# ShiqiYu/libfacedetection.train

Hardware: AMD Instinct MI355X
Metric: training images/sec, YuNet_n 320x320 bs=256/GPU (higher is better)
Workload: dtype f32; 1 GPU; YuNet_n 320x320 bs=256/GPU full training step, fp32 (64->64 backward GEMMs: two-way bf16 split -- measured against the exact-fp32 instruction: every output within 9e-6 of its tensor maximum, 50 SGD iterations end as far from the exact path as a last-bit perturbation of it does, tests/test_precision_gpu.py + profiles/r05_precision.json; the strictly-fp32 variant is timed in exact_fp32_bwd with --fu; parallelism=dp1, global_batch=256

## Files before the change

libfacedetection.train_amd/csrc/api.hip:

```cpp
#include <string.h>

#include "common.h"

namespace {

__global__ __launch_bounds__(256) void sgd_kernel(float* __restrict__ p, const float* __restrict__ g,
                                                  float* __restrict__ buf, long long n,
                                                  const float* __restrict__ lr_dev, float momentum, float undamped,
                                                  int nesterov, float wd, float gscale, int first) {
    const float lr = lr_dev[0];
    const long long i = (long long)blockIdx.x * 256 + threadIdx.x;
    if (i >= n) return;
    const float w = p[i];
    const float d = g[i] * gscale + wd * w;
    float step = d;
    if (momentum != 0.0f) {
        const float b = first ? d : buf[i] * momentum + undamped * d;
        buf[i] = b;
        step = nesterov ? d + momentum * b : b;
    }
    p[i] = w - lr * step;
}

__global__ void bn_batch_kernel(const int32_t* __restrict__ table, const double* __restrict__ stats_base,
                                float* __restrict__ rm, float* __restrict__ rv, float momentum,
                                float* __restrict__ grad_base, int mode) {
    const int32_t* t = table + blockIdx.x * 7;
    const int C = t[1], count = t[2], slots = t[6];
    const double* st = stats_base + t[0];
    for (int c = threadIdx.x; c < C; c += blockDim.x) {
        if (mode == 0) {
            const double inv = 1.0 / (double)count;
            const double mean = bn_sum(st, slots, C, c) * inv;
            double var = bn_sum(st, slots, C, C + c) * inv - mean * mean;
            var = var < 0.0 ? 0.0 : var;
            const double unb = count > 1 ? var * ((double)count / (double)(count - 1)) : var;
            float* m = rm + t[3];
            float* v = rv + t[3];
            m[c] = (1.0f - momentum) * m[c] + momentum * (float)mean;
            v[c] = (1.0f - momentum) * v[c] + momentum * (float)unb;
        } else if (mode == 1) {
            grad_base[t[5] + c] = (float)bn_sum(st, slots, C, c);
            grad_base[t[4] + c] = (float)bn_sum(st, slots, C, C + c);
        } else {
            double* w = const_cast<double*>(st);
            const double m = (double)rm[t[3] + c], v = (double)rv[t[3] + c];
            w[c] = m * (double)count;
            w[C + c] = (v + m * m) * (double)count;
            for (int k = 1; k < slots; ++k) w[k * 2 * C + c] = 0.0, w[k * 2 * C + C + c] = 0.0;
        }
    }
}

}

extern "C" int yunet_bn_batch(const int32_t* table, int n, const double* stats_base,
                              float* running_mean, float* running_var, float momentum,
                              float* grad_base, int mode, void* stream) {
    if (n < 1) return YUNET_EINVAL;
    hipLaunchKernelGGL(bn_batch_kernel, dim3(n), dim3(64), 0, (hipStream_t)stream, table, stats_base,
                       running_mean, running_var, momentum, grad_base, mode);
    return hip_status();
}

__global__ __launch_bounds__(256) void add_kernel(const float* __restrict__ a, const float* __restrict__ b,
                                                  float* __restrict__ out, size_t n, int vec) {
    const size_t i = (size_t)blockIdx.x * 256 + threadIdx.x;
    if (vec) {
        if (i < n / 4) {
            const float4 x = reinterpret_cast<const float4*>(a)[i], y = reinterpret_cast<const float4*>(b)[i];
            reinterpret_cast<float4*>(out)[i] = make_float4(x.x + y.x, x.y + y.y, x.z + y.z, x.w + y.w);
        } else if (i - n / 4 < n % 4) {
            const size_t k = (n / 4) * 4 + (i - n / 4);
            out[k] = a[k] + b[k];
        }
    } else if (i < n) {
        out[i] = a[i] + b[i];
    }
}

extern "C" int yunet_add(const float* a, const float* b, float* out, size_t n, void* stream) {
    if (!a || !b || !out) return YUNET_EINVAL;
    if (n == 0) return 0;
    const int vec = ((reinterpret_cast<uintptr_t>(a) | reinterpret_cast<uintptr_t>(b) | reinterpret_cast<uintptr_t>(out)) & 15) == 0;
    const size_t threads = vec ? n / 4 + n % 4 : n;
    const size_t blocks = (threads + 255) / 256;
    if (blocks > 0x7fffffffull) return YUNET_EINVAL;
    hipLaunchKernelGGL(add_kernel, dim3((unsigned)blocks), dim3(256), 0, (hipStream_t)stream, a, b, out, n, vec);
    return hip_status();
}

extern "C" int yunet_sgd_step_ex(float* params, const float* grads, float* momentum_buf, int64_t n,
                                 const float* lr_dev, float momentum, float dampening, int nesterov,
                                 float weight_decay, float grad_scale, int first_step, void* stream) {
    if (n < 1 || !params || !grads || !lr_dev) return YUNET_EINVAL;
    if (momentum != 0.0f && !momentum_buf) return YUNET_EINVAL;
    if (nesterov && (momentum <= 0.0f || dampening != 0.0f)) return YUNET_EINVAL;
    const long long blocks = (n + 255) / 256;
    if (blocks > 0x7fffffffll) return YUNET_EINVAL;
    hipLaunchKernelGGL(sgd_kernel, dim3((unsigned)blocks), dim3(256), 0, (hipStream_t)stream, params, grads,
                       momentum_buf, (long long)n, lr_dev, momentum, 1.0f - dampening, nesterov ? 1 : 0, weight_decay,
                       grad_scale, first_step);
    return hip_status();
}

extern "C" int yunet_sgd_step(float* params, const float* grads, float* momentum_buf, int64_t n,
                              const float* lr_dev, float momentum, float weight_decay,
                              float grad_scale, int first_step, void* stream) {
    return yunet_sgd_step_ex(params, grads, momentum_buf, n, lr_dev, momentum, 0.0f, 0, weight_decay, grad_scale,
                             first_step, stream);
}

YunetOptions& yunet_options() {
    static YunetOptions o = [] {
        auto env = [](const char* k, int dflt) {
            const char* e = getenv(k);
            return e ? atoi(e) : dflt;
        };
        YunetOptions v;
        v.no_pack = getenv("YUNET_NO_PACK") ? 1 : 0;
        v.bwd_fp32mma = getenv("YUNET_BWD_FP32MMA") ? 1 : 0;
        v.bwd64_nw = env("YUNET_BWD64_NW", 0);
        v.ew_grid = env("YUNET_EW_GRID", 768);
        v.fwd_blocks_per_cu = env("YUNET_DP_FWD_BLOCKS_PER_CU", 0);
        v.fwd64s = env("YUNET_FWD64S", 2);
        v.fwd64s_rows = env("YUNET_FWD64S_ROWS", 0);
        v.bwd16s = env("YUNET_BWD16S", 1);
        v.bwd16s_rows = env("YUNET_BWD16S_ROWS", 0);
        v.stem_mma = env("YUNET_STEM_MMA", 1);
        v.fwd16s = env("YUNET_FWD16S", 1);
        v.upadd_coarse = env("YUNET_UPADD_COARSE", 1);
        v.bwd32_split = env("YUNET_BWD32_SPLIT", 1);
        v.assign_v2 = env("YUNET_ASSIGN_V2", 1);
        v.fwd_group = env("YUNET_FWD_GROUP", 1);
        v.oneshot_timeout_ms = env("YUNET_ONESHOT_TIMEOUT_MS", 120000);
        if (v.bwd64_nw != 4 && v.bwd64_nw != 8) v.bwd64_nw = 0;
        if (v.ew_grid < 1) v.ew_grid = 768;
        return v;
    }();
    return o;
}
int yunet_option_assign_v2() { return yunet_options().assign_v2; }
extern "C" int yunet_set_option(const char* name, int value) {
    YunetOptions& o = yunet_options();
    int* slot = nullptr;
    if (!name) return YUNET_EINVAL;
    if (!strcmp(name, "no_pack")) slot = &o.no_pack;
    else if (!strcmp(name, "bwd_fp32mma")) slot = &o.bwd_fp32mma;
    else if (!strcmp(name, "bwd64_nw")) slot = &o.bwd64_nw;
    else if (!strcmp(name, "ew_grid")) slot = &o.ew_grid;
    else if (!strcmp(name, "fwd_blocks_per_cu")) slot = &o.fwd_blocks_per_cu;
    else if (!strcmp(name, "fwd64s")) slot = &o.fwd64s;
    else if (!strcmp(name, "fwd64s_rows")) slot = &o.fwd64s_rows;
    else if (!strcmp(name, "bwd16s")) slot = &o.bwd16s;
    else if (!strcmp(name, "bwd16s_rows")) slot = &o.bwd16s_rows;
    else if (!strcmp(name, "stem_mma")) slot = &o.stem_mma;
    else if (!strcmp(name, "fwd16s")) slot = &o.fwd16s;
    else if (!strcmp(name, "upadd_coarse")) slot = &o.upadd_coarse;
    else if (!strcmp(name, "bwd32_split")) slot = &o.bwd32_split;
    else if (!strcmp(name, "assign_v2")) slot = &o.assign_v2;
    else if (!strcmp(name, "fwd_group")) slot = &o.fwd_group;
    else if (!strcmp(name, "oneshot_timeout_ms")) slot = &o.oneshot_timeout_ms;
    if (!slot || value < 0) return YUNET_EINVAL;
    if (slot == &o.bwd64_nw && value != 0 && value != 4 && value != 8) return YUNET_EINVAL;
    if (slot == &o.ew_grid && value == 0) value = 768;
    const int prev = *slot;
    *slot = value;
    return prev;
}

extern "C" {
int yunet_stem_fwd_bf16(const float*, const float*, const float*, float*, double*, int, int, int, int, void*);
int yunet_stem_bwd_bf16(const float*, const float*, const float*, const YunetBN*, float*, int, int, int, int, int, void*);
int yunet_dp_fwd_bf16(const YunetDP*, void*);
int yunet_dp_fwd_group_bf16(const YunetDP* const*, int, void*);
int yunet_dp_bwd_bf16(const YunetDP*, void*);
int yunet_pool_fwd_bf16(const float*, const YunetBN*, float*, int, int, int, int, void*);
int yunet_pool_bwd_bf16(const float*, const YunetBN*, const float*, float*, int, int, int, int, int, void*);
int yunet_upadd_fwd_bf16(const float*, const YunetBN*, const float*, const YunetBN*, float*, int, int, int, int, void*);
int yunet_upadd_bwd_bf16(const float*, const YunetBN*, const float*, const YunetBN*, const float*, float*, int, float*,
                         int, int, int, int, int, void*);
}

static int g_lanes_on = 1;
struct LaneSet {
    bool ready;
    hipStream_t side[YUNET_MAX_LANES];
    hipEvent_t fork_ev, join_ev[YUNET_MAX_LANES];
};
static constexpr int kMaxDevices = 16;
static thread_local LaneSet t_lanes[kMaxDevices];
static LaneSet* lanes_get() {
    int dev = -1;
    if (hipGetDevice(&dev) != hipSuccess || dev < 0 || dev >= kMaxDevices) return nullptr;
    LaneSet& s = t_lanes[dev];
    if (s.ready) return &s;
    for (int l = 0; l < YUNET_MAX_LANES; ++l) {
        if (hipStreamCreateWithFlags(&s.side[l], hipStreamNonBlocking) != hipSuccess) return nullptr;
        if (hipEventCreateWithFlags(&s.join_ev[l], hipEventDisableTiming) != hipSuccess) return nullptr;
    }
    if (hipEventCreateWithFlags(&s.fork_ev, hipEventDisableTiming) != hipSuccess) return nullptr;
    s.ready = true;
    return &s;
}
extern "C" int yunet_exec_lanes(int enable) {
    const int prev = g_lanes_on;
    g_lanes_on = enable ? 1 : 0;
    return prev;
}

extern "C" int yunet_exec(const YunetOp* ops, int n_ops, void* main_stream) {
    unsigned open_lanes = 0;
    LaneSet* ls = nullptr;
    for (int k = 0; k < n_ops; ++k) {
        const YunetOp& o = ops[k];
        int rc = 0;
        void* stream = main_stream;
        if (o.opcode == YUNET_OP_FORK || o.opcode == YUNET_OP_JOIN) {
            if (!g_lanes_on) continue;
            if (!ls && !(ls = lanes_get())) return YUNET_EINVAL * 1000 - k;
            const unsigned mask = (unsigned)o.i[0] & ((1u << (YUNET_MAX_LANES + 1)) - 2u);
            if (o.opcode == YUNET_OP_FORK) {
                if (hipEventRecord(ls->fork_ev, (hipStream_t)main_stream) != hipSuccess) return YUNET_EINVAL * 1000 - k;
                for (int l = 1; l <= YUNET_MAX_LANES; ++l)
                    if (mask & (1u << l)) hipStreamWaitEvent(ls->side[l - 1], ls->fork_ev, 0);
                open_lanes |= mask;
            } else {
                for (int l = 1; l <= YUNET_MAX_LANES; ++l)
                    if (mask & (1u << l)) {
                        hipEventRecord(ls->join_ev[l - 1], ls->side[l - 1]);
                        hipStreamWaitEvent((hipStream_t)main_stream, ls->join_ev[l - 1], 0);
                    }
                open_lanes &= ~mask;
            }
            continue;
        }
        const int lane = o.i[YUNET_OP_LANE];
        if (g_lanes_on && lane > 0) {
            if (lane > YUNET_MAX_LANES || !(open_lanes & (1u << lane)) || !ls) return YUNET_EINVAL * 1000 - k;
            stream = (void*)ls->side[lane - 1];
        }
        switch (o.opcode) {
            case YUNET_OP_STEM_FWD:
                if (o.i[4] > 0) {
                    rc = o.i[11] == YUNET_BF16 ? YUNET_EINVAL
                                               : yunet_stem_fwd_det((const float*)o.p[0], (const float*)o.p[1], (const float*)o.p[2], (float*)o.p[3],
                                                                    (double*)o.p[4], o.i[4], o.i[0], o.i[1], o.i[2], o.i[3], stream);
                    break;
                }
                rc = (o.i[11] == YUNET_BF16 ? yunet_stem_fwd_bf16 : yunet_stem_fwd)((const float*)o.p[0], (const float*)o.p[1], (const float*)o.p[2],
                                    (float*)o.p[3], (double*)o.p[4], o.i[0], o.i[1], o.i[2], o.i[3],
                                    stream);
                break;
            case YUNET_OP_STEM_BWD:
                if (o.p[4] && o.p[5] && yunet_options().stem_mma) {
                    rc = yunet_stem_bwd_rz((const float*)o.p[0], (const float*)o.p[4], (const float*)o.p[5], (const float*)o.p[2],
                                           &o.bn[0], (float*)o.p[3], o.i[4], o.i[0], o.i[1], o.i[2], o.i[3], stream);
                    break;
                }
                rc = (o.i[11] == YUNET_BF16 ? yunet_stem_bwd_bf16 : yunet_stem_bwd)((const float*)o.p[0], (const float*)o.p[1], (const float*)o.p[2],
                                    &o.bn[0], (float*)o.p[3], o.i[4], o.i[0], o.i[1], o.i[2], o.i[3],
                                    stream);
                break;
            case YUNET_OP_DP_FWD: {
                const int g = o.i[YUNET_OP_GROUP];
                if (g >= 2 && g <= YUNET_DP_GROUP_MAX && k + g <= n_ops) {
                    const YunetDP* units[YUNET_DP_GROUP_MAX];
                    bool ok = true;
                    for (int j = 0; j < g; ++j) {
                        const YunetOp& oj = ops[k + j];
                        ok = ok && oj.opcode == YUNET_OP_DP_FWD && oj.i[YUNET_OP_LANE] == lane && oj.dp.x_dtype == o.dp.x_dtype;
                        units[j] = &oj.dp;
                    }
                    if (!ok) return YUNET_EINVAL * 1000 - k;
                    rc = o.dp.x_dtype == YUNET_BF16 ? yunet_dp_fwd_group_bf16(units, g, stream) : yunet_dp_fwd_group(units, g, stream);
                    if (rc == 0) k += g - 1;
                    break;
                }
                rc = o.dp.x_dtype == YUNET_BF16 ? yunet_dp_fwd_bf16(&o.dp, stream) : yunet_dp_fwd(&o.dp, stream);
                break;
            }
            case YUNET_OP_DP_BWD:
                rc = o.dp.x_dtype == YUNET_BF16 ? yunet_dp_bwd_bf16(&o.dp, stream) : yunet_dp_bwd(&o.dp, stream);
                break;
            case YUNET_OP_POOL_FWD:
                rc = (o.i[11] == YUNET_BF16 ? yunet_pool_fwd_bf16 : yunet_pool_fwd)((const float*)o.p[0], &o.bn[0], (float*)o.p[1], o.i[0], o.i[1],
                                    o.i[2], o.i[3], stream);
                break;
            case YUNET_OP_POOL_BWD:
                rc = (o.i[11] == YUNET_BF16 ? yunet_pool_bwd_add_bf16 : yunet_pool_bwd_add)(
                    (const float*)o.p[0], &o.bn[0], (const float*)o.p[1], (const float*)o.p[3], (float*)o.p[2], o.i[4], o.i[0],
                    o.i[1], o.i[2], o.i[3], stream);
                break;
            case YUNET_OP_UPADD_FWD:
                rc = (o.i[11] == YUNET_BF16 ? yunet_upadd_fwd_bf16 : yunet_upadd_fwd)((const float*)o.p[0], &o.bn[0], (const float*)o.p[1], &o.bn[1],
                                     (float*)o.p[2], o.i[0], o.i[1], o.i[2], o.i[3], stream);
                break;
            case YUNET_OP_UPADD_BWD:
                rc = (o.i[11] == YUNET_BF16 ? yunet_upadd_bwd_bf16 : yunet_upadd_bwd)((const float*)o.p[0], &o.bn[0], (const float*)o.p[1], &o.bn[1],
                                     (const float*)o.p[2], (float*)o.p[3], o.i[4], (float*)o.p[4],
                                     o.i[5], o.i[0], o.i[1], o.i[2], o.i[3], stream);
                break;
            case YUNET_OP_BN_RUNNING:
                rc = yunet_bn_update_running((const double*)o.p[0], (float*)o.p[1], (float*)o.p[2],
                                             o.i[0], o.i[1], o.f[0], stream);
                break;
            case YUNET_OP_BN_PARAM_GRAD:
                rc = yunet_bn_param_grad((const double*)o.p[0], (float*)o.p[1], (float*)o.p[2], o.i[0],
                                         o.i[1], stream);
                break;
            case YUNET_OP_REDUCE_PARTIALS:
                rc = yunet_reduce_partials((const float*)o.p[0], o.i[0], o.i[1], (float*)o.p[1],
                                           o.i[2], stream);
                break;
// ... 64 lines not shown
```

libfacedetection.train_amd/csrc/common.h:

```cpp
#pragma once
#include <hip/hip_runtime.h>
#include <stdint.h>
#include <stdlib.h>

#include "../../include/yunet_hip.h"

#define CONV_BLOCKS 1024

typedef float f32x4 __attribute__((ext_vector_type(4)));
typedef unsigned int u32x4 __attribute__((ext_vector_type(4)));
typedef unsigned int u32x2 __attribute__((ext_vector_type(2)));

#ifdef YUNET_ACT_BF16
typedef unsigned short act_t;
typedef u32x2 act_raw4;
#define ACT_SUFFIX(name) name##_bf16
#define YUNET_ACT_DTYPE YUNET_BF16
#else
typedef float act_t;
typedef u32x4 act_raw4;
#define ACT_SUFFIX(name) name
#define YUNET_ACT_DTYPE YUNET_F32
#endif
#define ACT_B ((unsigned)sizeof(act_t))
// ... 18 lines not shown
#else
    return act_raw4{__float_as_uint(v.x), __float_as_uint(v.y), __float_as_uint(v.z), __float_as_uint(v.w)};
#endif
}
__device__ __forceinline__ float act_round(float v) {
#ifdef YUNET_ACT_BF16
    return __uint_as_float(pack_bf16x2(v, 0.0f) << 16);
#else
    return v;
#endif
}
constexpr int ST_AUX = 0;
constexpr int DX_AUX = 2;
template <int AUX = 0, typename R>
__device__ __forceinline__ act_raw4 act_bufld4(R rsrc, unsigned byte_off) {
#ifdef YUNET_ACT_BF16
    return __builtin_amdgcn_raw_buffer_load_b64(rsrc, byte_off, 0, AUX);
#else
    return __builtin_amdgcn_raw_buffer_load_b128(rsrc, byte_off, 0, AUX);
#endif
}
template <typename R>
__device__ __forceinline__ void act_bufst4(R rsrc, unsigned byte_off, const float4 v) {
#ifdef YUNET_ACT_BF16
    __builtin_amdgcn_raw_buffer_store_b64(act_pack(v), rsrc, byte_off, 0, ST_AUX);
#else
    __builtin_amdgcn_raw_buffer_store_b128(act_pack(v), rsrc, byte_off, 0, ST_AUX);
#endif
}
__device__ __forceinline__ float4 act_ld4(const act_t* p) {
    return act_unpack(*reinterpret_cast<const act_raw4*>(p));
}
__device__ __forceinline__ void act_st4(act_t* p, const float4 v) {
    *reinterpret_cast<act_raw4*>(p) = act_pack(v);
}

__device__ __forceinline__ int first_tile() {
    const int g = (int)gridDim.x, b = (int)blockIdx.x;
    if ((g & 7) == 0) return (b & 7) * (g >> 3) + (b >> 3);
    return b;
}

__device__ __forceinline__ f32x4 mfma16(float a, float b, f32x4 c) {
    return __builtin_amdgcn_mfma_f32_16x16x4f32(a, b, c, 0, 0, 0);
}

struct BNCoef {
    float mean, scale, beta, invstd;
    float mean_lo;
};
__device__ __forceinline__ double bn_sum(const double* __restrict__ s, int slots, int C, int i) {
    double v[8];
#pragma unroll
    for (int k = 0; k < 8; ++k) v[k] = s[(k < slots ? k : 0) * 2 * C + i];
#pragma unroll
    for (int k = 1; k < 8; ++k) v[k] = k < slots ? v[k] : 0.0;
    double r = ((v[0] + v[1]) + (v[2] + v[3])) + ((v[4] + v[5]) + (v[6] + v[7]));
    for (int k = 8; k < slots; ++k) r += s[k * 2 * C + i];
    return r;
}
__device__ __forceinline__ double* bn_slot(const double* base, int slots, int C) {
    return const_cast<double*>(base) + (slots > 1 ? (int)(blockIdx.x % (unsigned)slots) * 2 * C : 0);
}
__device__ __forceinline__ BNCoef bn_coef(const YunetBN& bn, int C, int c) {
    const double inv = 1.0 / (double)bn.count;
    const double mean = bn_sum(bn.stats, bn.slots, C, c) * inv;
    double var = bn_sum(bn.stats, bn.slots, C, C + c) * inv - mean * mean;
    var = var < 0.0 ? 0.0 : var;
    BNCoef k;
    k.mean = (float)mean;
    k.mean_lo = (float)(mean - (double)k.mean);
    k.invstd = (float)(1.0 / sqrt(var + (double)bn.eps));
    k.scale = bn.gamma[c] * k.invstd;
    k.beta = bn.beta[c];
    return k;
}
__device__ __forceinline__ void bn_table_fill(float* tab, const YunetBN& bn, int C, int tid) {
    if (tid < C) {
        const BNCoef k = bn_coef(bn, C, tid);
        tab[tid] = k.mean; tab[C + tid] = k.scale; tab[2 * C + tid] = k.beta; tab[3 * C + tid] = k.invstd;
        tab[4 * C + tid] = k.mean_lo;
    }
}
__device__ __forceinline__ void bn_table_get(const float* tab, int C, int c0, BNCoef (&k)[4]) {
#pragma unroll
    for (int i = 0; i < 4; ++i) {
        k[i].mean = tab[c0 + i]; k[i].scale = tab[C + c0 + i]; k[i].beta = tab[2 * C + c0 + i];
        k[i].invstd = tab[3 * C + c0 + i]; k[i].mean_lo = tab[4 * C + c0 + i];
    }
}

struct BNBwd {
    float mean, invstd, k1, c1, c2;
    float mean_lo, c1_lo;
};
__device__ __forceinline__ BNBwd bn_bwd_coef(const YunetBN& bn, int C, int c) {
    const BNCoef f = bn_coef(bn, C, c);
    const double inv = 1.0 / (double)bn.count;
    BNBwd k;
    k.mean = f.mean;
    k.invstd = f.invstd;
    k.k1 = f.scale;
    const double c1 = bn_sum(bn.bstats, bn.slots, C, c) * inv;
    k.c1 = (float)c1;
    k.c1_lo = (float)(c1 - (double)k.c1);
    k.c2 = (float)(bn_sum(bn.bstats, bn.slots, C, C + c) * inv);
    k.mean_lo = f.mean_lo;
    return k;
}

struct BNFold {
    float a, b, dh, dl;
};
__device__ __forceinline__ BNFold bn_fold(const BNBwd& k) {
    BNFold f;
    f.a = k.k1;
    f.b = (float)(-(double)k.k1 * (double)k.c2 * (double)k.invstd);
    const double D = -(double)f.a * ((double)k.c1 + (double)k.c1_lo) - (double)f.b * ((double)k.mean + (double)k.mean_lo);
    f.dh = (float)D;
    f.dl = (float)(D - (double)f.dh);
    return f;
}
__device__ __forceinline__ float bn_dz_folded(float dy, float z, float a, float b, float dh, float dl) {
    return fmaf(a, dy, fmaf(b, z, dh)) + dl;
}

__device__ __forceinline__ float bn_center(float x, float mean_hi, float mean_lo) {
    return (x - mean_hi) - mean_lo;
}
__device__ __forceinline__ float bn_dz(float dy, float z, float mean_hi, float mean_lo, float invstd,
                                       float k1, float c1_hi, float c1_lo, float c2) {
    return k1 * (((dy - c1_hi) - c1_lo) - bn_center(z, mean_hi, mean_lo) * invstd * c2);
}

__device__ __forceinline__ float bnrelu(float x, float mean, float scale, float beta) {
    return fmaxf(fmaf(x - mean, scale, beta), 0.0f);
}

struct YunetOptions {
    int no_pack;
    int bwd_fp32mma;
    int bwd64_nw;
    int ew_grid;
    int fwd_blocks_per_cu;
    int fwd64s;
    int fwd64s_rows;
    int bwd16s;
    int bwd16s_rows;
    int fwd16s;
    int stem_mma;
    int bwd32_split;
    int upadd_coarse;
    int fwd_group;
    int assign_v2;
    int oneshot_timeout_ms;
};
YunetOptions& yunet_options();
int yunet_option_assign_v2();

#include <atomic>
constexpr int YUNET_MAX_DEVICES = 16;
struct PerDevice {
    std::atomic<int> v[YUNET_MAX_DEVICES];
};
inline int yunet_device_index() {
    int dev = 0;
    if (hipGetDevice(&dev) != hipSuccess || dev < 0 || dev >= YUNET_MAX_DEVICES) return -1;
    return dev;
}
template <typename F>
inline int per_device(PerDevice& slots, F&& compute) {
    const int dev = yunet_device_index();
    if (dev < 0) return compute();
    int v = slots.v[dev].load(std::memory_order_acquire);
    if (v == 0) {
        v = compute();
        if (v > 0) slots.v[dev].store(v, std::memory_order_release);
    }
    return v;
}
inline int yunet_cu_count() {
    static PerDevice cus;
    return per_device(cus, [] {
        int dev = 0, n = 0;
        if (hipGetDevice(&dev) != hipSuccess ||
            hipDeviceGetAttribute(&n, hipDeviceAttributeMultiprocessorCount, dev) != hipSuccess || n < 1)
            return 256;
        return n;
    });
}

#ifdef __HIPCC__
template <int COUNT, int NT, typename F>
__device__ __forceinline__ void staged_table(const float* __restrict__ src, int tid, F&& put) {
    constexpr int IT = (COUNT + NT - 1) / NT;
    constexpr bool EXACT = COUNT % NT == 0;
    float v[IT];
#pragma unroll
    for (int k = 0; k < IT; ++k) {
        const int i = tid + k * NT;
        v[k] = (EXACT || i < COUNT) ? src[i] : 0.0f;
    }
#pragma unroll
    for (int k = 0; k < IT; ++k) {
        const int i = tid + k * NT;
        if (EXACT || i < COUNT) put(i, v[k]);
    }
}
#endif


struct PackGeom {
    int on, H, W, ph, pw, R, N, CH, CW;
    float inv_ph, inv_pw;
};
static inline PackGeom make_pack(int N, int H, int W) {
    PackGeom g;
    g.on = (H <= 20 && W <= 20 && N >= 4) ? 1 : 0;
    g.H = H; g.W = W; g.N = N;
    g.ph = H + 1; g.pw = W + 1;
    g.R = N < 16 ? N : 16;
    g.CW = g.R * g.pw;
    g.CH = ((N + g.R - 1) / g.R) * g.ph;
    g.inv_ph = 1.0f / (float)g.ph;
    g.inv_pw = 1.0f / (float)g.pw;
    return g;
}
static inline PackGeom dp_pack_geom(int N, int H, int W) {
    PackGeom g = make_pack(N, H, W);
    if (yunet_options().no_pack) g.on = 0;
    return g;
}
static inline bool dp_use_pack(int N, int H, int W, int cin, int cout) {
    return cin == 64 && (cout == 64 || cout == 16) && dp_pack_geom(N, H, W).on;
}
static inline bool dp_use_pack_bwd(int N, int H, int W, int cin, int cout) {
    return dp_use_pack(N, H, W, cin, cout);
}
static inline bool dp_pack_fits(const PackGeom& g, long long x_img_stride, long long z_img_stride) {
    const long long lim = 1ll << 30;
    return !g.on || ((long long)g.N * x_img_stride < lim && (long long)g.N * z_img_stride < lim);
}
__device__ __forceinline__ bool pk_locate(const PackGeom& g, int Y, int X, int& n, int& y, int& x) {
    if ((unsigned)Y >= (unsigned)g.CH || (unsigned)X >= (unsigned)g.CW) return false;
    const int iy = (int)(((float)Y + 0.5f) * g.inv_ph), ix = (int)(((float)X + 0.5f) * g.inv_pw);
    y = Y - iy * g.ph;
    x = X - ix * g.pw;
    n = iy * g.R + ix;
    return y < g.H && x < g.W && n < g.N;
}

__device__ __forceinline__ void atomic_add_f64(double* p, double v) {
    __hip_atomic_fetch_add(p, v, __ATOMIC_RELAXED, __HIP_MEMORY_SCOPE_AGENT);
}

__device__ __forceinline__ void bn_det_add(const double* base, int C, int i, double v) {
    double* p = const_cast<double*>(base) + (size_t)(1 + blockIdx.x) * 2 * C + i;
    *p += v;
}
static inline bool bn_det_fits(const YunetBN& bn, int grid) { return YUNET_DET_ROWS(bn.det_rows) >= grid && bn.slots <= 1; }
static inline bool bn_det_fast(const YunetBN& bn) { return YUNET_DET_ROWS(bn.det_rows) && (bn.det_rows & YUNET_DET_FAST); }

static inline int hip_status() { return -(int)hipGetLastError(); }

int ACT_SUFFIX(launch_dp_fwd64s)(const YunetDP* d, hipStream_t stream);
int ACT_SUFFIX(launch_dp_fwd64s_group)(const YunetDP* const* ds, int n, hipStream_t stream);
int ACT_SUFFIX(launch_dp_bwd16s)(const YunetDP* d, hipStream_t stream);
int ACT_SUFFIX(launch_dp_bwd64)(const YunetDP* d, int nw, hipStream_t stream);
int ACT_SUFFIX(launch_dp_fwd16s)(const YunetDP* d, hipStream_t stream);
int ACT_SUFFIX(launch_stem_fwd_mma)(const float* img, const float* w, const float* b, float* z, double* stats, int N, int H, int W,
                                    hipStream_t stream);
int launch_stem_fwd_mma_det(const float* img, const float* w, const float* b, float* z, double* stats, int det_rows, int N, int H,
                            int W, hipStream_t stream);
int launch_stem_bwd_mma(const float* img, const float* w, const float* b, const float* dy, const YunetBN* bn, float* partials,
                        int blocks, int N, int H, int W, hipStream_t stream);
```

libfacedetection.train_amd/csrc/conv_fwd.hip:

```cpp
#include <cstdlib>

#include <stdlib.h>

#include "common.h"

namespace {

#define STEM_TW 32
#define STEM_TH 16
#define STEM_PX 2
__global__ __launch_bounds__(256) void stem_fwd_kernel(const float* __restrict__ img,
                                                       const float* __restrict__ w,
                                                       const float* __restrict__ b,
                                                       act_t* __restrict__ z,
                                                       double* __restrict__ stats, int N, int H,
                                                       int W) {
    constexpr int PH = 2 * STEM_TH + 1;
    constexpr int PW4 = (2 * STEM_TW + 8) / 4;
    constexpr int PWS = PW4 * 4 + 1;
    constexpr int NLD = (3 * PH * PW4 + 255) / 256;
    __shared__ float s_patch[3 * PH * PWS];
    __shared__ __attribute__((aligned(16))) float s_w[27][16];
    __shared__ double s_stat[32];
    const int tid = threadIdx.x;
// ... 551 lines not shown
    for (long long e = (long long)blockIdx.x * 256 + threadIdx.x; e < total;
         e += (long long)gridDim.x * 256) {
        long long pix = e / C4;
        const int ox = (int)(pix % Wo);
        pix /= Wo;
        const int oy = (int)(pix % Ho), n = (int)(pix / Ho);
        float4 m = make_float4(0, 0, 0, 0);
#pragma unroll
        for (int dy = 0; dy < 2; ++dy)
#pragma unroll
            for (int dx = 0; dx < 2; ++dx) {
                const float4 v = act_ld4(z + (((size_t)n * H + 2 * oy + dy) * W + 2 * ox + dx) * C + c4 * 4);
                m.x = fmaxf(m.x, bnrelu(v.x, k[0].mean, k[0].scale, k[0].beta));
                m.y = fmaxf(m.y, bnrelu(v.y, k[1].mean, k[1].scale, k[1].beta));
                m.z = fmaxf(m.z, bnrelu(v.z, k[2].mean, k[2].scale, k[2].beta));
                m.w = fmaxf(m.w, bnrelu(v.w, k[3].mean, k[3].scale, k[3].beta));
            }
        act_st4(out + e * 4, m);
    }
}

__global__ __launch_bounds__(256) void upadd_fwd_kernel(const act_t* __restrict__ za, YunetBN bna,
                                                        const act_t* __restrict__ zb, YunetBN bnb,
                                                        act_t* __restrict__ out, int N, int H, int W,
                                                        int C) {
    const int C4 = C / 4, Hb = H / 2, Wb = W / 2;
    const long long total = (long long)N * H * W * C4;
    const int c4 = threadIdx.x % C4;
    __shared__ float s_ta[5 * 64], s_tb[5 * 64];
    bn_table_fill(s_ta, bna, C, threadIdx.x);
    bn_table_fill(s_tb, bnb, C, threadIdx.x);
    __syncthreads();
    BNCoef ka[4], kb[4];
    bn_table_get(s_ta, C, c4 * 4, ka);
    bn_table_get(s_tb, C, c4 * 4, kb);
    for (long long e = (long long)blockIdx.x * 256 + threadIdx.x; e < total;
         e += (long long)gridDim.x * 256) {
        long long pix = e / C4;
        const int x = (int)(pix % W);
        pix /= W;
        const int y = (int)(pix % H), n = (int)(pix / H);
        const float4 a = act_ld4(za + e * 4);
        const float4 b = act_ld4(zb + (((size_t)n * Hb + y / 2) * Wb + x / 2) * C + c4 * 4);
        float av[4] = {a.x, a.y, a.z, a.w}, bv[4] = {b.x, b.y, b.z, b.w}, o[4];
#pragma unroll
        for (int i = 0; i < 4; ++i)
            o[i] = bnrelu(av[i], ka[i].mean, ka[i].scale, ka[i].beta) +
                   bnrelu(bv[i], kb[i].mean, kb[i].scale, kb[i].beta);
        act_st4(out + e * 4, make_float4(o[0], o[1], o[2], o[3]));
    }
}

#ifndef YUNET_ACT_BF16
__global__ void bn_running_kernel(const double* __restrict__ stats, float* __restrict__ rm,
                                  float* __restrict__ rv, int C, int count, float momentum) {
    const int c = blockIdx.x * blockDim.x + threadIdx.x;
    if (c >= C) return;
    const double inv = 1.0 / (double)count;
    const double mean = stats[c] * inv;
    double var = stats[C + c] * inv - mean * mean;
    var = var < 0.0 ? 0.0 : var;
    const double unb = count > 1 ? var * ((double)count / (double)(count - 1)) : var;
    rm[c] = (1.0f - momentum) * rm[c] + momentum * (float)mean;
    rv[c] = (1.0f - momentum) * rv[c] + momentum * (float)unb;
}
#endif

inline int ew_grid(long long total) {
    long long b = (total + 255) / 256;
    return (int)(b < 1 ? 1 : (b > 2048 ? 2048 : b));
}

}

extern "C" int ACT_SUFFIX(yunet_stem_fwd)(const float* img, const float* w, const float* b, float* z,
                                          double* stats, int N, int H, int W, int cmid, void* stream) {
    if (cmid != 16 || (H & 1) || (W & 1)) return YUNET_EINVAL;
    if (yunet_options().stem_mma) return ACT_SUFFIX(launch_stem_fwd_mma)(img, w, b, z, stats, N, H, W, (hipStream_t)stream);
    const int tiles = N * ((W / 2 + STEM_TW - 1) / STEM_TW) * ((H / 2 + STEM_TH - 1) / STEM_TH);
    const int grid = tiles < 768 ? tiles : 768;
    hipLaunchKernelGGL(stem_fwd_kernel, dim3(grid), dim3(256), 0, (hipStream_t)stream, img, w, b,
                       reinterpret_cast<act_t*>(z), stats, N, H, W);
    return hip_status();
}

#ifndef YUNET_ACT_BF16
extern "C" int yunet_stem_fwd_det(const float* img, const float* w, const float* b, float* z, double* stats, int det_rows,
                                  int N, int H, int W, int cmid, void* stream) {
    if (cmid != 16 || (H & 1) || (W & 1) || !stats) return YUNET_EINVAL;
    return launch_stem_fwd_mma_det(img, w, b, z, stats, det_rows, N, H, W, (hipStream_t)stream);
}
#endif

extern "C" int ACT_SUFFIX(yunet_dp_fwd)(const YunetDP* d, void* stream) {
    hipStream_t s = (hipStream_t)stream;
    if (d->x_dtype != YUNET_ACT_DTYPE) return YUNET_EINVAL;
    if (d->z_dtype != YUNET_ACT_DTYPE && !(d->cout == 16 && d->z_dtype == YUNET_F32)) return YUNET_EINVAL;
    if (d->in_transform != YUNET_T_IDENTITY && d->in_transform != YUNET_T_BNRELU) return YUNET_EINVAL;
    const bool det = d->out_has_bn && YUNET_DET_ROWS(d->out_bn.det_rows);
    const bool det_fast = det && bn_det_fast(d->out_bn) && YUNET_ACT_DTYPE == YUNET_F32;
    const bool fwd16s = (!det || det_fast) && d->cin == 16 && (d->cout == 16 || (d->cout == 64 && !d->pool_out)) && d->z_dtype == YUNET_ACT_DTYPE &&
                        !d->prof && yunet_options().fwd16s &&
                        (!d->pool_out || (yunet_dp_pool_fusion_ok(d->N, d->H, d->W, 16, 16) && d->out_bn.gamma && d->pool_idx &&
                                          !(reinterpret_cast<uintptr_t>(d->pool_idx) & 3)));
    if (!d->z && !(fwd16s && d->pool_out)) return YUNET_EINVAL;
    if (det) {
#ifndef YUNET_ACT_BF16
        if (d->z_dtype != YUNET_ACT_DTYPE || !d->out_bn.stats) return YUNET_EINVAL;
        if (det_fast) {
            if (fwd16s) return launch_dp_fwd16s(d, s);
            const bool pool_ok = d->pool_out && yunet_dp_pool_fusion_ok(d->N, d->H, d->W, d->cin, d->cout) && d->out_bn.gamma &&
                                 d->pool_idx && !(reinterpret_cast<uintptr_t>(d->pool_idx) & 3);
            const bool packed_tile = dp_use_pack(d->N, d->H, d->W, d->cin, d->cout) && yunet_options().fwd64s < 2;
            if (d->cin == 64 && d->cout == 64 && (unsigned long long)d->prof < 64ull && yunet_options().fwd64s &&
                (d->pool_out ? pool_ok : !packed_tile))
                return launch_dp_fwd64s(d, s);
        }
        if (d->pool_out) {
            if (!yunet_dp_pool_fusion_ok(d->N, d->H, d->W, d->cin, d->cout) || !d->out_bn.gamma || !d->pool_idx ||
                (reinterpret_cast<uintptr_t>(d->pool_idx) & 3))
                return YUNET_EINVAL;
            if (d->cin == 16) return launch_dp_fwd<16, 16, 16, 32, false, true, true>(d, s);
            if (d->cin == 32) return launch_dp_fwd<32, 64, 8, 16, false, true, true>(d, s);
            return launch_dp_fwd<64, 64, 8, 16, false, true, true>(d, s);
        }
        if (d->cin == 16 && d->cout == 16 && d->W >= 64 && d->H >= 32) return launch_dp_fwd<16, 16, 16, 32, false, false, true>(d, s);
        if (dp_use_pack(d->N, d->H, d->W, d->cin, d->cout) && d->cout == 64) return launch_dp_fwd<64, 64, 8, 16, true, false, true>(d, s);
#define DP_CASE(ci, co) \
    if (d->cin == ci && d->cout == co) return launch_dp_fwd<ci, co, 8, 16, false, false, true>(d, s);
        DP_CASE(16, 16)
        DP_CASE(16, 32)
        DP_CASE(16, 64)
        DP_CASE(32, 32)
        DP_CASE(32, 64)
        DP_CASE(64, 64)
#undef DP_CASE
#endif
        return YUNET_EINVAL;
    }
    if (fwd16s) return ACT_SUFFIX(launch_dp_fwd16s)(d, s);
    if (d->pool_out) {
        if (!yunet_dp_pool_fusion_ok(d->N, d->H, d->W, d->cin, d->cout) || !d->out_bn.gamma || !d->pool_idx ||
            (reinterpret_cast<uintptr_t>(d->pool_idx) & 3))
            return YUNET_EINVAL;
        if (d->cin == 16) return launch_dp_fwd<16, 16, 16, 32, false, true>(d, s);
        if (d->cin == 32) return launch_dp_fwd<32, 64, 8, 16, false, true>(d, s);
        if ((unsigned long long)d->prof < 64ull && yunet_options().fwd64s && d->z_dtype == YUNET_ACT_DTYPE) return ACT_SUFFIX(launch_dp_fwd64s)(d, s);
        return launch_dp_fwd<64, 64, 8, 16, false, true>(d, s);
    }
#define DP_CASE(ci, co) \
    if (d->cin == ci && d->cout == co) return launch_dp_fwd<ci, co, 8, 16>(d, s);
    if (d->cin == 16 && d->cout == 16 && d->W >= 64 && d->H >= 32)
        return launch_dp_fwd<16, 16, 16, 32>(d, s);
    if (dp_use_pack(d->N, d->H, d->W, d->cin, d->cout) && !(d->cout == 64 && d->z_dtype == YUNET_ACT_DTYPE && yunet_options().fwd64s >= 2))
        return d->cout == 64 ? launch_dp_fwd<64, 64, 8, 16, true>(d, s) : launch_dp_fwd<64, 16, 8, 16, true>(d, s);
    if (d->cin == 64 && d->cout == 64 && d->z_dtype == YUNET_ACT_DTYPE && (unsigned long long)d->prof < 64ull && yunet_options().fwd64s)
        return ACT_SUFFIX(launch_dp_fwd64s)(d, s);
    DP_CASE(16, 16)
    DP_CASE(16, 32)
    DP_CASE(16, 64)
    DP_CASE(32, 32)
    DP_CASE(32, 64)
    DP_CASE(64, 64)
    DP_CASE(64, 16)
#undef DP_CASE
    return YUNET_EINVAL;
}

extern "C" int ACT_SUFFIX(yunet_dp_fwd_group)(const YunetDP* const* units, int n, void* stream) {
    if (!units || n < 1 || n > YUNET_DP_GROUP_MAX) return YUNET_EINVAL;
    bool one_grid = n >= 2 && yunet_options().fwd_group != 0;
    for (int i = 0; i < n && one_grid; ++i) {
        const YunetDP* d = units[i];
        one_grid = d && !(d->out_has_bn && YUNET_DET_ROWS(d->out_bn.det_rows)) &&
                   d->x_dtype == YUNET_ACT_DTYPE && d->z_dtype == YUNET_ACT_DTYPE && d->cin == 64 && d->cout == 64 &&
                   d->z && !d->pool_out && !d->prof && yunet_options().fwd64s != 0 &&
                   (d->in_transform == YUNET_T_IDENTITY || d->in_transform == YUNET_T_BNRELU) &&
                   !(dp_use_pack(d->N, d->H, d->W, d->cin, d->cout) && yunet_options().fwd64s < 2);
    }
    if (one_grid) return ACT_SUFFIX(launch_dp_fwd64s_group)(units, n, (hipStream_t)stream);
    for (int i = 0; i < n; ++i) {
        if (!units[i]) return YUNET_EINVAL;
        const int rc = ACT_SUFFIX(yunet_dp_fwd)(units[i], stream);
        if (rc) return rc;
    }
    return 0;
}

extern "C" int ACT_SUFFIX(yunet_pool_fwd)(const float* z, const YunetBN* bn, float* out, int N, int H, int W,
                                          int C, void* stream) {
    if ((H & 1) || (W & 1) || (C & 3) || (256 % (C / 4)) || C > 64) return YUNET_EINVAL;
    const long long total = (long long)N * (H / 2) * (W / 2) * (C / 4);
    hipLaunchKernelGGL(pool_fwd_kernel, dim3(ew_grid(total)), dim3(256), 0, (hipStream_t)stream,
                       reinterpret_cast<const act_t*>(z), *bn, reinterpret_cast<act_t*>(out), N, H, W, C);
    return hip_status();
}

extern "C" int ACT_SUFFIX(yunet_upadd_fwd)(const float* za, const YunetBN* bna, const float* zb,
                                           const YunetBN* bnb, float* out, int N, int H, int W, int C,
                                           void* stream) {
    if ((H & 1) || (W & 1) || (C & 3) || (256 % (C / 4)) || C > 64) return YUNET_EINVAL;
    const long long total = (long long)N * H * W * (C / 4);
    hipLaunchKernelGGL(upadd_fwd_kernel, dim3(ew_grid(total)), dim3(256), 0, (hipStream_t)stream,
                       reinterpret_cast<const act_t*>(za), *bna, reinterpret_cast<const act_t*>(zb), *bnb,
                       reinterpret_cast<act_t*>(out), N, H, W, C);
    return hip_status();
}

#ifndef YUNET_ACT_BF16
extern "C" int yunet_bn_update_running(const double* stats, float* running_mean,
                                       float* running_var, int C, int count, float momentum,
                                       void* stream) {
    hipLaunchKernelGGL(bn_running_kernel, dim3((C + 63) / 64), dim3(64), 0, (hipStream_t)stream,
                       stats, running_mean, running_var, C, count, momentum);
    return hip_status();
}

extern "C" int yunet_conv_blocks(void) { return CONV_BLOCKS; }
extern "C" int yunet_abi_version(void) { return YUNET_ABI_VERSION; }
#endif
```

Measured before the change: 58770 images/sec.

## Add dedicated MFMA kernel for 64->16 detection-head depthwise-pointwise forward

```diff
diff --git a/libfacedetection.train_amd/csrc/api.hip b/libfacedetection.train_amd/csrc/api.hip
--- a/libfacedetection.train_amd/csrc/api.hip
+++ b/libfacedetection.train_amd/csrc/api.hip
@@ -133,6 +133,7 @@
         v.bwd32_split = env("YUNET_BWD32_SPLIT", 1);
         v.assign_v2 = env("YUNET_ASSIGN_V2", 1);
         v.fwd_group = env("YUNET_FWD_GROUP", 1);
+        v.head_kernels = env("YUNET_HEAD_KERNELS", 1);
         v.oneshot_timeout_ms = env("YUNET_ONESHOT_TIMEOUT_MS", 120000);
         if (v.bwd64_nw != 4 && v.bwd64_nw != 8) v.bwd64_nw = 0;
         if (v.ew_grid < 1) v.ew_grid = 768;
@@ -160,6 +161,7 @@
     else if (!strcmp(name, "bwd32_split")) slot = &o.bwd32_split;
     else if (!strcmp(name, "assign_v2")) slot = &o.assign_v2;
     else if (!strcmp(name, "fwd_group")) slot = &o.fwd_group;
+    else if (!strcmp(name, "head_kernels")) slot = &o.head_kernels;
     else if (!strcmp(name, "oneshot_timeout_ms")) slot = &o.oneshot_timeout_ms;
     if (!slot || value < 0) return YUNET_EINVAL;
     if (slot == &o.bwd64_nw && value != 0 && value != 4 && value != 8) return YUNET_EINVAL;
diff --git a/libfacedetection.train_amd/csrc/common.h b/libfacedetection.train_amd/csrc/common.h
--- a/libfacedetection.train_amd/csrc/common.h
+++ b/libfacedetection.train_amd/csrc/common.h
@@ -194,6 +194,7 @@
     int bwd32_split;
     int upadd_coarse;
     int fwd_group;
+    int head_kernels;
     int assign_v2;
     int oneshot_timeout_ms;
 };
@@ -309,6 +310,8 @@
 int ACT_SUFFIX(launch_dp_fwd64s_group)(const YunetDP* const* ds, int n, hipStream_t stream);
 int ACT_SUFFIX(launch_dp_bwd16s)(const YunetDP* d, hipStream_t stream);
 int ACT_SUFFIX(launch_dp_bwd64)(const YunetDP* d, int nw, hipStream_t stream);
+bool dp_fwd_head_fits(const YunetDP* d);
+int launch_dp_fwd_head(const YunetDP* d, hipStream_t stream);
 int ACT_SUFFIX(launch_dp_fwd16s)(const YunetDP* d, hipStream_t stream);
 int ACT_SUFFIX(launch_stem_fwd_mma)(const float* img, const float* w, const float* b, float* z, double* stats, int N, int H, int W,
                                     hipStream_t stream);
diff --git a/libfacedetection.train_amd/csrc/conv_fwd.hip b/libfacedetection.train_amd/csrc/conv_fwd.hip
--- a/libfacedetection.train_amd/csrc/conv_fwd.hip
+++ b/libfacedetection.train_amd/csrc/conv_fwd.hip
@@ -727,6 +727,11 @@
     if (d->cin == ci && d->cout == co) return launch_dp_fwd<ci, co, 8, 16>(d, s);
     if (d->cin == 16 && d->cout == 16 && d->W >= 64 && d->H >= 32)
         return launch_dp_fwd<16, 16, 16, 32>(d, s);
+#ifndef YUNET_ACT_BF16
+    if (d->cin == 64 && d->cout == 16 && !d->out_has_bn && d->z_dtype == YUNET_F32 && !d->prof && yunet_options().head_kernels &&
+        dp_fwd_head_fits(d))
+        return launch_dp_fwd_head(d, s);
+#endif
     if (dp_use_pack(d->N, d->H, d->W, d->cin, d->cout) && !(d->cout == 64 && d->z_dtype == YUNET_ACT_DTYPE && yunet_options().fwd64s >= 2))
         return d->cout == 64 ? launch_dp_fwd<64, 64, 8, 16, true>(d, s) : launch_dp_fwd<64, 16, 8, 16, true>(d, s);
     if (d->cin == 64 && d->cout == 64 && d->z_dtype == YUNET_ACT_DTYPE && (unsigned long long)d->prof < 64ull && yunet_options().fwd64s)
diff --git a/libfacedetection.train_amd/csrc/conv_fwd_head.hip b/libfacedetection.train_amd/csrc/conv_fwd_head.hip
--- /dev/null
+++ b/libfacedetection.train_amd/csrc/conv_fwd_head.hip
@@ -0,0 +1,201 @@
+#include "common.h"
+
+namespace {
+namespace fh {
+constexpr int CI = 64, CO = 16, TW = 14, PX = 16, WAVES = 4, NTHR = 64 * WAVES;
+constexpr int SPX = PX + 2;
+constexpr int SLOT = SPX * CO;
+constexpr int BLOCKS_PER_CU = 3;
+}
+
+typedef __bf16 bf16x8_h __attribute__((ext_vector_type(8)));
+
+__device__ __forceinline__ float med3h(float a, float b, float c) { return __builtin_amdgcn_fmed3f(a, b, c); }
+
+struct Split3 {
+    unsigned h, m, l;
+};
+__device__ __forceinline__ Split3 split3(float a0, float a1) {
+    Split3 s;
+    s.h = pack_bf16x2(a0, a1);
+    const float r0 = a0 - __uint_as_float(s.h << 16), r1 = a1 - __uint_as_float(s.h & 0xffff0000u);
+    s.m = pack_bf16x2(r0, r1);
+    s.l = pack_bf16x2(r0 - __uint_as_float(s.m << 16), r1 - __uint_as_float(s.m & 0xffff0000u));
+    return s;
+}
+
+__global__ __launch_bounds__(fh::NTHR, fh::BLOCKS_PER_CU) void dp_fwd_head_kernel(const YunetDP d, const int R) {
+    using namespace fh;
+    __shared__ __attribute__((aligned(16))) float s_p[WAVES * SLOT];
+    __shared__ __attribute__((aligned(16))) float s_w2[9 * CO];
+    __shared__ __attribute__((aligned(16))) float s_b2[CO];
+    __shared__ __attribute__((aligned(16))) float s_sc[CI];
+    __shared__ __attribute__((aligned(16))) float s_sh[CI];
+    const int tid = threadIdx.x, lane = tid & 63;
+    const int wid = __builtin_amdgcn_readfirstlane(tid >> 6);
+    const int l15 = lane & 15, g = lane >> 4;
+    const int H = d.H, W = d.W;
+    const bool bn_in = d.in_transform == YUNET_T_BNRELU;
+
+    u32x4 wh[2], wm[2], wl[2];
+    {
+        float4 ra[2], rb[2];
+#pragma unroll
+        for (int kb = 0; kb < 2; ++kb) {
+            ra[kb] = *reinterpret_cast<const float4*>(d.w_pw + l15 * CI + 32 * kb + 8 * g);
+            rb[kb] = *reinterpret_cast<const float4*>(d.w_pw + l15 * CI + 32 * kb + 8 * g + 4);
+        }
+#pragma unroll
+        for (int kb = 0; kb < 2; ++kb) {
+            const float w8[8] = {ra[kb].x, ra[kb].y, ra[kb].z, ra[kb].w, rb[kb].x, rb[kb].y, rb[kb].z, rb[kb].w};
+#pragma unroll
+            for (int q = 0; q < 4; ++q) {
+                const Split3 sp = split3(w8[2 * q], w8[2 * q + 1]);
+                wh[kb][q] = sp.h; wm[kb][q] = sp.m; wl[kb][q] = sp.l;
+            }
+        }
+    }
+    const float4 b1v = *reinterpret_cast<const float4*>(d.b_pw + 4 * g);
+    staged_table<CO * 9, NTHR>(d.w_dw, tid, [&](int i, float w) { s_w2[(i % 9) * CO + i / 9] = w; });
+    if (tid < CO) s_b2[tid] = d.b_dw[tid];
+    if (tid < CI) {
+        float sc = 1.0f, sh = 0.0f;
+        if (bn_in) {
+            const BNCoef k = bn_coef(d.in_bn, CI, tid);
+            sc = k.scale;
+            sh = (float)((double)k.beta - ((double)k.mean + (double)k.mean_lo) * (double)k.scale);
+        }
+        s_sc[tid] = sc; s_sh[tid] = sh;
+    }
+    for (int i = tid; i < WAVES * 2 * CO; i += NTHR) s_p[(i / (2 * CO)) * SLOT + PX * CO + i % (2 * CO)] = 0.0f;
+    __syncthreads();
+
+    const float relu_floor = bn_in ? 0.0f : -__builtin_inff();
+    float* pslot = s_p + wid * SLOT;
+    const int strips = (W + TW - 1) / TW, bands = (H + R - 1) / R;
+    const int tasks_img = strips * bands, ntasks = d.N * tasks_img;
+    const unsigned xbytes = (unsigned)(H * W * CI) * 4u, zbytes = (unsigned)(H * W * CO) * 4u;
+    const int cq = lane & 3, c = lane >> 2;
+    const int total_waves = (int)gridDim.x * WAVES;
+    const float4 b2 = *reinterpret_cast<const float4*>(s_b2 + cq * 4);
+
+    for (int t = first_tile() * WAVES + wid; t < ntasks; t += total_waves) {
+        const int n = t / tasks_img, rr = t - n * tasks_img;
+        const int band = rr / strips, strip = rr - band * strips;
+        const int y0 = band * R, y1 = (y0 + R < H) ? y0 + R : H;
+        const int xs = strip * TW;
+        const int col = xs - 1 + l15;
+        const bool colv = (unsigned)col < (unsigned)W;
+        const float cap = colv ? __builtin_inff() : 0.0f;
+        const auto r_x = __builtin_amdgcn_make_buffer_rsrc(const_cast<float*>(d.x) + (size_t)n * d.x_img_stride, 0, xbytes, 0x00020000);
+        const auto r_z = __builtin_amdgcn_make_buffer_rsrc(d.z + (size_t)n * d.z_img_stride, 0, zbytes, 0x00020000);
+        const unsigned xlane = colv ? (unsigned)(col * CI + 8 * g) * 4u : xbytes;
+        const f32x4 bias = colv ? f32x4{b1v.x, b1v.y, b1v.z, b1v.w} : f32x4{0.f, 0.f, 0.f, 0.f};
+        const int xc = xs + c;
+        const unsigned zlane = (c < TW && xc < W) ? (unsigned)(xc * CO + cq * 4) * 4u : zbytes;
+        const int rs = y0 > 0 ? y0 - 1 : 0, re = y1 < H ? y1 : H - 1;
+        u32x4 xr[4];
+        auto issue = [&](int y) {
+            const unsigned o = xlane + (unsigned)(y * W * CI) * 4u;
+            xr[0] = __builtin_amdgcn_raw_buffer_load_b128(r_x, o, 0, 0);
+            xr[1] = __builtin_amdgcn_raw_buffer_load_b128(r_x, o + 16, 0, 0);
+            xr[2] = __builtin_amdgcn_raw_buffer_load_b128(r_x, o + 128, 0, 0);
+            xr[3] = __builtin_amdgcn_raw_buffer_load_b128(r_x, o + 144, 0, 0);
+        };
+        issue(rs);
+        float4 oa = b2, ob = b2;
+        auto emit_row = [&](int yy, const float4& v) {
+            const u32x4 bits = {__float_as_uint(v.x), __float_as_uint(v.y), __float_as_uint(v.z), __float_as_uint(v.w)};
+            __builtin_amdgcn_raw_buffer_store_b128(bits, r_z, (unsigned)(yy * W * CO) * 4u + zlane, 0, ST_AUX);
+        };
+
+#pragma unroll 1
+        for (int r = rs; r <= re; ++r) {
+            u32x4 bh[2], bm[2], bl[2];
+#pragma unroll
+            for (int kb = 0; kb < 2; ++kb) {
+                const float4 s0 = *reinterpret_cast<const float4*>(s_sc + 32 * kb + 8 * g);
+                const float4 s1 = *reinterpret_cast<const float4*>(s_sc + 32 * kb + 8 * g + 4);
+                const float4 h0 = *reinterpret_cast<const float4*>(s_sh + 32 * kb + 8 * g);
+                const float4 h1 = *reinterpret_cast<const float4*>(s_sh + 32 * kb + 8 * g + 4);
+                const float sc[8] = {s0.x, s0.y, s0.z, s0.w, s1.x, s1.y, s1.z, s1.w};
+                const float sh[8] = {h0.x, h0.y, h0.z, h0.w, h1.x, h1.y, h1.z, h1.w};
+                float a[8];
+#pragma unroll
+                for (int e = 0; e < 4; ++e) {
+                    a[e] = med3h(fmaf(__uint_as_float(xr[2 * kb][e]), sc[e], sh[e]), relu_floor, cap);
+                    a[4 + e] = med3h(fmaf(__uint_as_float(xr[2 * kb + 1][e]), sc[4 + e], sh[4 + e]), relu_floor, cap);
+                }
+#pragma unroll
+                for (int q = 0; q < 4; ++q) {
+                    const Split3 sp = split3(a[2 * q], a[2 * q + 1]);
+                    bh[kb][q] = sp.h; bm[kb][q] = sp.m; bl[kb][q] = sp.l;
+                }
+            }
+            if (r < re) issue(r + 1);
+
+            f32x4 acc0 = bias, acc1 = f32x4{0.f, 0.f, 0.f, 0.f};
+#define HEAD_MFMA(acc, W, B) \
+    acc = __builtin_amdgcn_mfma_f32_16x16x32_bf16(__builtin_bit_cast(bf16x8_h, W), __builtin_bit_cast(bf16x8_h, B), acc, 0, 0, 0);
+            HEAD_MFMA(acc0, wh[0], bl[0]) HEAD_MFMA(acc1, wh[1], bl[1])
+            HEAD_MFMA(acc0, wl[0], bh[0]) HEAD_MFMA(acc1, wl[1], bh[1])
+            HEAD_MFMA(acc0, wm[0], bm[0]) HEAD_MFMA(acc1, wm[1], bm[1])
+            HEAD_MFMA(acc0, wh[0], bm[0]) HEAD_MFMA(acc1, wh[1], bm[1])
+            HEAD_MFMA(acc0, wm[0], bh[0]) HEAD_MFMA(acc1, wm[1], bh[1])
+            HEAD_MFMA(acc0, wh[0], bh[0]) HEAD_MFMA(acc1, wh[1], bh[1])
+#undef HEAD_MFMA
+            const f32x4 acc = acc0 + acc1;
+            __builtin_amdgcn_fence(__ATOMIC_RELEASE, "wavefront");
+            __builtin_amdgcn_wave_barrier();
+            *reinterpret_cast<f32x4*>(pslot + l15 * CO + 4 * g) = acc;
+            __builtin_amdgcn_fence(__ATOMIC_RELEASE, "wavefront");
+            __builtin_amdgcn_wave_barrier();
+            __builtin_amdgcn_fence(__ATOMIC_ACQUIRE, "wavefront");
+
+            const float* pp = pslot + c * CO + cq * 4;
+            const float4 pl = *reinterpret_cast<const float4*>(pp);
+            const float4 pm = *reinterpret_cast<const float4*>(pp + CO);
+            const float4 pr = *reinterpret_cast<const float4*>(pp + 2 * CO);
+            float4 w[9];
+#pragma unroll
+            for (int k = 0; k < 9; ++k) w[k] = *reinterpret_cast<const float4*>(s_w2 + k * CO + cq * 4);
+            float4 o = oa, mid = ob, top = b2;
+#define TAP(o, k, v)                                                                        \
+    o.x = fmaf(v.x, w[k].x, o.x); o.y = fmaf(v.y, w[k].y, o.y); o.z = fmaf(v.z, w[k].z, o.z); \
+    o.w = fmaf(v.w, w[k].w, o.w);
+            TAP(o, 6, pl) TAP(o, 7, pm) TAP(o, 8, pr)
+            TAP(mid, 3, pl) TAP(mid, 4, pm) TAP(mid, 5, pr)
+            TAP(top, 0, pl) TAP(top, 1, pm) TAP(top, 2, pr)
+#undef TAP
+            oa = mid; ob = top;
+            if (r - 1 >= y0) emit_row(r - 1, o);
+        }
+        if (y1 == H) emit_row(H - 1, oa);
+    }
+}
+
+int head_rows(int N, int H, int W, int waves) {
+    const int strips = (W + fh::TW - 1) / fh::TW;
+    int R = H;
+    while (R > 8 && (long long)N * strips * ((H + R - 1) / R) < (long long)waves) R = (R + 1) / 2;
+    while (R > 2 && (long long)N * strips * ((H + R - 1) / R) < (long long)waves / 4) R = (R + 1) / 2;
+    return R;
+}
+
+}
+
+bool dp_fwd_head_fits(const YunetDP* d) {
+    return (long long)d->H * d->W * fh::CI * 4 < (1ll << 31);
+}
+
+int launch_dp_fwd_head(const YunetDP* d, hipStream_t stream) {
+    if (d->x_dtype != YUNET_F32 || d->z_dtype != YUNET_F32 || !d->z || !dp_fwd_head_fits(d)) return YUNET_EINVAL;
+    int grid = yunet_cu_count() * fh::BLOCKS_PER_CU;
+    const int R = head_rows(d->N, d->H, d->W, grid * fh::WAVES);
+    const long long tasks = (long long)d->N * ((d->W + fh::TW - 1) / fh::TW) * ((d->H + R - 1) / R);
+    const long long need = (tasks + fh::WAVES - 1) / fh::WAVES;
+    if (need < grid) grid = (int)need;
+    if (grid < 1) return YUNET_EINVAL;
+    hipLaunchKernelGGL(dp_fwd_head_kernel, dim3(grid), dim3(fh::NTHR), 0, stream, *d, R);
+    return hip_status();
+}
```

Result: no change. 59120 images/sec, median of 6 (+0.6%).
